# Black-Phoenix/CUDA-SfM

Hardware: AMD Instinct MI355X
Metric: RANSAC E-matrix hypotheses/sec (8-point, fused scoring), inlier-mask parity vs CPU oracle (higher is better)
Workload: dtype f32

## Files before the change

### cuda-sfm_amd/csrc/prefilter_lds.hpp

```cpp
#pragma once
#include "prefilter_record.hpp"

namespace sfm {

constexpr int kPfTileMax = 1024;
constexpr int kPfWaves = 16;
constexpr int kPfRing = 128;

constexpr int kPfERow = 10;
constexpr int kPfWaveBytes = 32 * kPfERow * 4 + 32 * 4;
template <int RULE> struct PfLds {
    static constexpr int kFragsPerBlock = RULE == kPfRuleG ? 3 : 2;
    static constexpr int kBlockBytes = kFragsPerBlock * 64 * 16;
    static constexpr int kFrag = 0;
    static constexpr int kTileMax = kPfTileMax;
    int staged, pts, ring, wave, next, lut, bytes;
    __host__ __device__ explicit PfLds(int tile, int ring_entries = kPfRing, int entry_bytes = 8)
    {
        staged = (tile + 63) & ~63;
        pts = kFrag + (staged / 32) * kBlockBytes;
        ring = pts + staged * 16;
        ring = (ring + ring_entries * entry_bytes - 1) & ~(ring_entries * entry_bytes - 1);
        wave = ring + kPfWaves * ring_entries * entry_bytes;
        next = wave + kPfWaves * kPfWaveBytes;
        lut = next + 16;
        bytes = lut + 32;
    }
};
static_assert(kPfRing * 8 == 1024, "ring slots are addressed with (offset & 1023) | base");

static inline int pf_tile_points(int ld, int tmax)
{
    const int ntiles = (ld + tmax - 1) / tmax;
    const int t = ((ld + ntiles - 1) / ntiles + 31) & ~31;
    return t < 32 ? 32 : t;
}

}
```

### cuda-sfm_amd/csrc/ransac_prefilter.hip

```cpp
#include "ransac_device.hpp"
#include "block_ops.hpp"
#include "prefilter_math.hpp"
#include "prefilter_record.hpp"
#include "prefilter_lds.hpp"

namespace sfm {

typedef float f16v __attribute__((ext_vector_type(16)));


__device__ constexpr int kPfESlot[9] = { 2, 6, 1, 3, 5, 7, 0, 4, 8 };
__device__ __forceinline__ uint32_t shift_in_reject(uint32_t rejected, float nt, float G)
{
    return __builtin_amdgcn_alignbit(rejected, __float_as_uint(fmaf(-nt, nt, G)), 31);
}

__device__ __forceinline__ uint32_t scan16(const f16v &nt, const f16v &G)
{
    uint32_t rejected = 0u;
#pragma unroll
    for (int r = 0; r < 16; ++r) rejected = shift_in_reject(rejected, nt[r], G[r]);
    return rejected;
}

__device__ __forceinline__ uint32_t scan16_band(const f16v &nt)
{
    uint32_t w = 0u;
#pragma unroll
    for (int r = 0; r < 16; ++r) w = __builtin_amdgcn_alignbit(w, __float_as_uint(nt[r]), 30);
    return w;
}

typedef uint32_t u6v __attribute__((ext_vector_type(6)));
constexpr uint32_t kPackM0 = 0x10410410u, kPackM1 = 0x04104104u;

__device__ __forceinline__ uint32_t pf_bfi(uint32_t m, uint32_t a, uint32_t b) { return __builtin_amdgcn_bitop3_b32(m, a, b, 0xCA); }

__device__ __forceinline__ uint32_t pack_reject_bits(const u6v &d)
{
    const uint32_t wa = pf_bfi(kPackM0 | kPackM1, pf_bfi(kPackM0, d[0], d[1]), d[2]);
    const uint32_t wb = pf_bfi(kPackM0 | kPackM1, pf_bfi(kPackM0, d[3], d[4]), d[5]);
    return pf_bfi(0x55555555u, wa, wb << 1);
}

typedef uint32_t u2v __attribute__((ext_vector_type(2)));
typedef float f4v __attribute__((ext_vector_type(4)));
typedef __attribute__((address_space(3))) u2v lds_u2;
typedef uint32_t u4v __attribute__((ext_vector_type(4)));
typedef __attribute__((address_space(3))) u4v lds_u4;
typedef __attribute__((address_space(3))) const f4v lds_cf4;
typedef __attribute__((address_space(3))) const float lds_cf;
typedef __attribute__((address_space(3))) int lds_i;
typedef __attribute__((address_space(3))) const h8 lds_ch8;
typedef __attribute__((address_space(3))) const v2f lds_cv2;
typedef __attribute__((address_space(3))) const unsigned char lds_cu8;

struct PfFrags { h8 n0, n1, t; };

__device__ __forceinline__ bool pf_exact_inlier(v2f p0, v2f p1, v2f p2, v2f p3, float e8, v2f xu, v2f yv, const ThrBand &band)
{
    const v2f e00 = { p3.x, p3.x }, e44 = { p3.y, p3.y }, e31 = { p1.y, p1.x };
    const v2f ab0 = __builtin_elementwise_fma(p1, yv, __builtin_elementwise_fma(e00, xu, p0));
    const v2f ab1 = __builtin_elementwise_fma(e44, yv, __builtin_elementwise_fma(e31, xu, p2));
    const float a2 = fmaf(p2.y, yv.x, fmaf(p0.y, xu.x, e8));
    const float nn = fmaf(yv.y, ab1.x, fmaf(xu.y, ab0.x, a2));
    const float n2 = nn * nn;
    const v2f dd = __builtin_elementwise_fma(ab1, ab1, ab0 * ab0);
    const float da = dd.x, db = dd.y;
    const float m = n2 * (da + db);
    const float tp = (da * db) * band.thr;
    const uint32_t mb = __float_as_uint(m), tb = __float_as_uint(tp);
    const uint32_t gap = __usad(mb, tb, 0u);
    const bool undecided = (gap < kBandUlps) || (tb < band.lo_bits) || (tb > band.hi_bits);
    bool in = m < tp;
    if (undecided) {
        const float t1 = (da == 0.0f) ? 0.0f : n2 / da;
        const float t2 = (db == 0.0f) ? 0.0f : n2 / db;
        in = (t1 + t2) < band.thr;
    }
    return in;
}

template <int RULE>
__device__ __forceinline__ PfFrags load_point_frags(lds_ch8 *frag_lane, int pb)
{
    lds_ch8 *p = frag_lane + pb * (PfLds<RULE>::kBlockBytes / 16);
    if (RULE != kPfRuleG) return PfFrags{ p[0], p[64], h8{} };
    return PfFrags{ p[0], p[64], p[128] };
}

template <int RULE>
__device__ __forceinline__ void mfma_step(const PfFrags &a, const PfFrags &b, f16v &G, f16v &nt)
{
    const f16v z = {};
    nt = __builtin_amdgcn_mfma_f32_32x32x16_f16(a.n0, b.n0, z, 0, 0, 0);
    if (RULE == kPfRuleG) G = __builtin_amdgcn_mfma_f32_32x32x16_f16(a.t, b.t, z, 0, 0, 0);
    nt = __builtin_amdgcn_mfma_f32_32x32x16_f16(a.n1, b.n1, nt, 0, 0, 0);
}

#define PF_SCHED_STEP()                                                 \
    do {                                                                \
        if (RULE != kPfRuleG) {                                         \
            __builtin_amdgcn_sched_group_barrier(0x008, 1, 0);          \
            __builtin_amdgcn_sched_group_barrier(0x002, 8, 0);          \
            __builtin_amdgcn_sched_group_barrier(0x008, 1, 0);          \
            __builtin_amdgcn_sched_group_barrier(0x002, 8, 0);          \
        } else {                                                        \
            __builtin_amdgcn_sched_group_barrier(0x008, 1, 0);          \
            __builtin_amdgcn_sched_group_barrier(0x002, 11, 0);         \
            __builtin_amdgcn_sched_group_barrier(0x008, 1, 0);          \
            __builtin_amdgcn_sched_group_barrier(0x002, 11, 0);         \
            __builtin_amdgcn_sched_group_barrier(0x008, 1, 0);          \
            __builtin_amdgcn_sched_group_barrier(0x002, 11, 0);         \
        }                                                               \
    } while (0)

constexpr int kPfVarTickets = 1;

constexpr int pf_score_waves_per_simd(int var, int rule, int fl2, int pipe, int wide, int prio)
{
    return (var == 0 && (rule == kPfRuleBandTile || rule == kPfRuleBandPack) && !fl2 && !pipe && !wide && !prio) ? 5 : 4;
}

template <int W, int VAR = 0, int RULE = kPfRuleBandTile, int FL2 = 0, int PIPE = 0, int WIDE = 0, int PRIO = 0>
__global__ __launch_bounds__(W * 64, pf_score_waves_per_simd(VAR, RULE, FL2, PIPE, WIDE, PRIO))
void ransac_score_prefilter(const float *__restrict__ X0, const float *__restrict__ X1, int ld, int n,
                            const float *__restrict__ Ecand, const PfRecord *__restrict__ recs, uint32_t h0, uint32_t count, float thr,
                            int dynamic, int tile,
                            int *__restrict__ counts, uint32_t *__restrict__ tick,
                            unsigned long long *best_key, unsigned long long *best_key2, unsigned long long *__restrict__ clk,
                            const unsigned long long *__restrict__ bound_word, const uint32_t *__restrict__ tile_boxes)
{
    extern __shared__ __attribute__((aligned(16))) unsigned char smem[];
    const int lane = threadIdx.x & 63;
    const int wave = __builtin_amdgcn_readfirstlane(threadIdx.x >> 6);
    const bool probe = clk && blockIdx.x == 0 && blockIdx.y == 0 && threadIdx.x == 0;
    unsigned long long c0 = 0, w0 = 0;
    if (clk && blockIdx.x == 0 && blockIdx.y == 0 && wave == 0) { c0 = clock64(); w0 = wall_clock64(); }
#if SFM_AB
    const uint32_t trace_blk = blockIdx.y * gridDim.x + blockIdx.x;
    unsigned long long *trace = (clk && trace_blk < (uint32_t)kTraceBlocks) ? clk + 8 + (size_t)trace_blk * kTraceWords : nullptr;
    if (trace && threadIdx.x == 0) {
        trace[0] = wall_clock64();
        trace[2] = ((unsigned long long)__builtin_amdgcn_s_getreg((20 << 0) | (0 << 6) | (31 << 11)) << 32) |
                   (unsigned long long)__builtin_amdgcn_s_getreg((4 << 0) | (0 << 6) | (31 << 11));
        trace[3] = ((unsigned long long)blockIdx.y << 32) | blockIdx.x;
    }
#define PF_PHASE(k) do { if (probe1) clk[k] = wall_clock64() - w0; } while (0)
#else
#define PF_PHASE(k) do { } while (0)
#endif
    const int half = lane >> 5, row = lane & 31;
    const uint32_t npass = (count + (uint32_t)kPfGroup - 1u) / (uint32_t)kPfGroup;
    const uint32_t nstatic = gridDim.x * (uint32_t)W;
    using LT = PfLds<RULE>;
    constexpr bool kBand = RULE != kPfRuleG, kTile = RULE == kPfRuleBandTile, kPack = RULE == kPfRuleBandPack || kTile;
    static_assert(!(FL2 && kPack) && !(VAR && kPack), "the recorded variants were built on the v_alignbit scan");
    constexpr int kRing = FL2 ? 256 : kPfRing;
    constexpr int kEnt = WIDE ? 16 : 8;
    static_assert(!WIDE || (kPack && !PIPE && !FL2), "wide entries: the packed scan's plain loop only");
    const LT L(tile, kRing, kEnt);
    float *etab = reinterpret_cast<float *>(smem + L.wave + wave * kPfWaveBytes);
    int *cnt = reinterpret_cast<int *>(etab + 32 * kPfERow);

    PfFrags afrag = {};
    uint32_t key0 = 0u;
    float rec_dn = 0.0f, rec_lin = 0.0f;
    float e_row[9] = {};
    auto fetch_pass = [&](uint32_t pass, PfFrags &af, uint32_t &k0, float (&e)[9], float &dn, float &lin) {
        const uint32_t hf = pass * (uint32_t)kPfGroup;
        const uint32_t h = hf + (uint32_t)min(row, (int)min((uint32_t)kPfGroup, count - hf) - 1);
        if (kTile) {
            const float *src = Ecand + 9 * (size_t)h;
#pragma unroll
            for (int k = 0; k < 9; ++k) e[k] = src[k];
            const uint4 rec = reinterpret_cast<const uint4 *>(recs)[h];
            k0 = rec.x; dn = __uint_as_float(rec.y); lin = __uint_as_float(rec.z);
            return;
        }
        const uint4 *r = reinterpret_cast<const uint4 *>(recs + h) + 2 * half;
        const uint4 r0 = r[0], r1 = r[1];
        if (kBand) pf_band_record_expand(r0, r1, half, af.n0, af.n1, k0);
        else pf_record_expand(r0, r1, half, af.n0, af.n1, af.t, k0);
        if (half == 0) {
            const float *src = Ecand + 9 * (size_t)h;
#pragma unroll
            for (int k = 0; k < 9; ++k) e[k] = src[k];
        }
    };
    auto install_rows = [&](const float (&e)[9]) {
        if (half == 0) {
#pragma unroll
            for (int k = 0; k < 9; ++k) etab[32 * k + row] = e[kPfESlot[k]];
            cnt[row] = 0;
        }
    };
    uint32_t ps = blockIdx.x * (uint32_t)W + (uint32_t)wave;
    bool have = ps < npass;
    if (have) { fetch_pass(ps, afrag, key0, e_row, rec_dn, rec_lin); install_rows(e_row); }

    SFM_PHASE("stage_tile");
    uint32_t *next_idx = reinterpret_cast<uint32_t *>(smem + L.next);
    if (threadIdx.x == 0) *next_idx = (uint32_t)W;
    if (kPack && threadIdx.x < 32) smem[L.lut + threadIdx.x] = (unsigned char)pf_pack_code((int)threadIdx.x);
    float pf_B = 0.0f;
    uint32_t bw[8] = {};
    uint32_t bw_lane = 0u;
    if (kTile) {
        pf_B = __uint_as_float((uint32_t)(__hip_atomic_load(reinterpret_cast<const uint32_t *>(bound_word), __ATOMIC_RELAXED, __HIP_MEMORY_SCOPE_AGENT)));
        bw_lane = __hip_atomic_load(tile_boxes + 8 * blockIdx.y + (lane & 7), __ATOMIC_RELAXED, __HIP_MEMORY_SCOPE_AGENT);
    }
    __syncthreads();
    const int tile_first = blockIdx.y * tile;
    for (int t = threadIdx.x; t < L.staged; t += W * 64) {
        const int p = tile_first + t;
        float u = 0.f, v = 0.f, x = 0.f, y = 0.f;
        const bool real = p < n && t < tile;
        if (kTile) {
            if (real) {
                const float4 q4 = reinterpret_cast<const float4 *>(X0)[p];
                u = q4.x; v = q4.y; x = q4.z; y = q4.w;
            }
        } else
        if (real) { u = X0[p]; v = X0[(size_t)ld + p]; x = X1[p]; y = X1[(size_t)ld + p]; }
        _Float16 bn[kPfSlots], bt[kPfSlotsT];
        prefilter_point_slots(u, v, x, y, real, bn, bt);
        reinterpret_cast<float4 *>(smem + L.pts)[t] = real ? make_float4(x, u, y, v) : make_float4(NAN, NAN, NAN, NAN);
        const int pb = t >> 5, col = t & 31;
        unsigned char *blk = smem + LT::kFrag + pb * LT::kBlockBytes;
#pragma unroll
        for (int ks = 0; ks < 2; ++ks)
#pragma unroll
            for (int hh = 0; hh < 2; ++hh) {
                h8 c;
#pragma unroll
                for (int j = 0; j < 8; ++j) c[j] = bn[ks * 16 + hh * 8 + j];
                *reinterpret_cast<h8 *>(blk + ks * 1024 + (hh * 32 + col) * 16) = c;
            }
        if (RULE == kPfRuleG) {
#pragma unroll
            for (int hh = 0; hh < 2; ++hh) {
                h8 c;
#pragma unroll
                for (int j = 0; j < 8; ++j) c[j] = bt[hh * 8 + j];
                *reinterpret_cast<h8 *>(blk + 2048 + (hh * 32 + col) * 16) = c;
            }
        }
    }
    __syncthreads();
    PfBox tbox = {};
    auto build_operands = [&](const float (&e)[9], uint32_t fl, float dn, float lin) {
        int half_l = half;
        float thr_l = thr, B_l = pf_B;
        asm volatile("" : "+v"(half_l), "+s"(thr_l), "+s"(B_l));
        pf_tile_operands(e, fl, dn, lin, thr_l, B_l, tbox, half_l, afrag.n0, afrag.n1);
        key0 = fl & kPfTileFlagScan;
    };
    if (kTile) {
#pragma unroll
        for (int k = 0; k < 8; ++k) bw[k] = (uint32_t)__builtin_amdgcn_readlane((int)bw_lane, k);
        pf_B = uniform(pf_B);
        tbox = pf_box_from_bits(bw, pf_B);
        tbox = PfBox{ uniform(tbox.xlo), uniform(tbox.xhi), uniform(tbox.ylo), uniform(tbox.yhi), uniform(tbox.ulo), uniform(tbox.uhi), uniform(tbox.vlo), uniform(tbox.vhi) };
        if (have) build_operands(e_row, key0, rec_dn, rec_lin);
    }
#if SFM_AB
    if (probe) clk[2] = wall_clock64() - w0;
#endif
    const int npb = (min(tile, ld - tile_first) + 31) >> 5;
    const int npp = (npb + 1) >> 1;
    const float4 *pts = reinterpret_cast<const float4 *>(smem + L.pts);
    lds_cf *etab_l = (lds_cf *)etab;
    lds_i *cnt_l = (lds_i *)cnt;
    lds_cu8 *lut_l = (lds_cu8 *)(smem + L.lut);
    const uint32_t ring_base = (uint32_t)(size_t)(__attribute__((address_space(3))) unsigned char *)(smem + L.ring) + (uint32_t)wave * (uint32_t)(kRing * kEnt);
    uint32_t ring_mask = (uint32_t)(kRing * kEnt - 1);
    asm("" : "+v"(ring_mask));
    auto ring_at = [&](uint32_t index8) {
        return (lds_u2 *)((__attribute__((address_space(3))) unsigned char *)0 + ((index8 & ring_mask) | ring_base));
    };
    auto ring_at16 = [&](uint32_t index16) {
        return (lds_u4 *)((__attribute__((address_space(3))) unsigned char *)0 + ((index16 & ring_mask) | ring_base));
    };
    lds_ch8 *frag_lane = (lds_ch8 *)(smem + LT::kFrag) + lane;
    const ThrBand band = make_band(thr);
    uint32_t passes_done = 0;

    while (have) {
        SFM_PHASE("pass_begin");
        const uint32_t h_first = ps * (uint32_t)kPfGroup;
        const int nvalid = (int)min((uint32_t)kPfGroup, count - h_first);
#if SFM_AB
        const bool probe1 = probe && passes_done == 0u;
#endif
        uint32_t ps_next = ps + nstatic;
        if (dynamic) {
            uint32_t got = 0u;
            if (lane == 0) got = atomicAdd(next_idx, 1u);
            got = (uint32_t)__builtin_amdgcn_readfirstlane((int)got);
            ps_next = (got / (uint32_t)W) * nstatic + blockIdx.x * (uint32_t)W + (got % (uint32_t)W);
        }
        {
            const bool scan = key0 != 0u;
            const unsigned long long sm = __ballot(scan);
            uint32_t todo = (uint32_t)sm | (uint32_t)(sm >> 32);
            uint32_t survive = 0u;
            while (todo) {
                const int r = __builtin_ctz(todo);
                todo &= todo - 1u;
                const float se[6] = { etab[6 * 32 + r], etab[2 * 32 + r], etab[r], etab[3 * 32 + r], etab[7 * 32 + r], etab[4 * 32 + r] };
                bool z = false;
                for (int j = 0; j < L.staged / 64; ++j) {
                    const float4 q = pts[j * 64 + lane];
                    z = z || prefilter_zero_divisor(se, q.x, q.z);
                }
                if (__ballot(z) != 0ull) survive |= 1u << r;
            }
            if (survive != 0u && ((survive >> row) & 1u)) {
                const h8 zero = {};
                afrag.n0 = zero; afrag.n1 = zero; afrag.t = zero;
                if (half) { afrag.n1[3] = (_Float16)1.0f; afrag.t[7] = (_Float16)0.0009765625f; }
            }
        }
        PF_PHASE(3);

        int head = 0, nq = 0;
        const uint32_t lane_tag = (uint32_t)(size_t)(lds_cf4 *)pts + (uint32_t)(row * 16) + (uint32_t)(half * 4);
        auto flush = [&](int m) {
            uint32_t rest = 0, tag = 0;
            if (PRIO == 2) __builtin_amdgcn_s_setprio(2);
            if (lane < m) {
                const u2v ent = *ring_at(((uint32_t)head + (uint32_t)lane) * 8u);
                tag = ent.y;
                const uint32_t surv = ent.x;
                const int b = __builtin_clz(surv);
                rest = surv & ~(0x80000000u >> b);
                int hl, sub;
                if (kPack) {
                    const uint32_t code = lut_l[b];
                    hl = (int)(code & 31u) + (int)(tag & 4u); sub = (int)(code >> 5);
                } else {
                    const int r = kBand ? b >> 1 : b & 15;
                    sub = kBand ? b & 1 : b >> 4;
                    hl = r + (r & 12) + (int)(tag & 4u);
                }
                if (hl < nvalid) {
                    const f4v q = *(lds_cf4 *)((__attribute__((address_space(3))) const unsigned char *)0 + ((tag & ~15u) + ((uint32_t)sub << 9)));
                    lds_cf *e = etab_l + hl;
                    const v2f p0 = { e[0], e[32] }, p1 = { e[64], e[96] }, p2 = { e[128], e[160] }, p3 = { e[192], e[224] };
                    const float e8 = e[256];
                    if (pf_exact_inlier(p0, p1, p2, p3, e8, v2f{ q.x, q.y }, v2f{ q.z, q.w }, band))
                        __hip_atomic_fetch_add(cnt_l + hl, 1, __ATOMIC_RELAXED, __HIP_MEMORY_SCOPE_WORKGROUP);
                }
            }
            const unsigned long long more = __ballot(rest != 0u);
            if (more) {
                const int slot = __builtin_amdgcn_mbcnt_hi((uint32_t)(more >> 32), __builtin_amdgcn_mbcnt_lo((uint32_t)more, 0u));
                if (rest) *ring_at(((uint32_t)(head + nq) + (uint32_t)slot) * 8u) = u2v{ rest, tag };
            }
            head = (head + m) & (kRing - 1);
            nq += __builtin_popcountll(more) - m;
            if (PRIO == 2) __builtin_amdgcn_s_setprio(0);
        };
        auto flush_w = [&](int m) {
            uint32_t ra = 0, rb = 0, tag = 0;
            if (lane < m) {
                const u4v ent = *ring_at16(((uint32_t)head + (uint32_t)lane) * 16u);
                tag = ent.z;
                const bool second = ent.x == 0u;
                const uint32_t surv = second ? ent.y : ent.x;
                const int b = __builtin_clz(surv);
                const uint32_t left = surv & ~(0x80000000u >> b);
                ra = second ? 0u : left; rb = second ? left : ent.y;
                const uint32_t code = lut_l[b];
                const int hl = (int)(code & 31u) + (int)(tag & 4u);
                if (hl < nvalid) {
                    const f4v q = *(lds_cf4 *)((__attribute__((address_space(3))) const unsigned char *)0 + ((tag & ~15u) + ((code >> 5) << 9) + (second ? 1024u : 0u)));
                    lds_cf *e = etab_l + hl;
                    const v2f p0 = { e[0], e[32] }, p1 = { e[64], e[96] }, p2 = { e[128], e[160] }, p3 = { e[192], e[224] };
                    const float e8 = e[256];
                    if (pf_exact_inlier(p0, p1, p2, p3, e8, v2f{ q.x, q.y }, v2f{ q.z, q.w }, band))
                        __hip_atomic_fetch_add(cnt_l + hl, 1, __ATOMIC_RELAXED, __HIP_MEMORY_SCOPE_WORKGROUP);
                }
            }
            const unsigned long long more = __ballot((ra | rb) != 0u);
            if (more) {
                const int slot = __builtin_amdgcn_mbcnt_hi((uint32_t)(more >> 32), __builtin_amdgcn_mbcnt_lo((uint32_t)more, 0u));
                if ((ra | rb) != 0u) *ring_at16(((uint32_t)(head + nq) + (uint32_t)slot) * 16u) = u4v{ ra, rb, tag, 0u };
            }
            head = (head + m) & (kRing - 1);
            nq += __builtin_popcountll(more) - m;
        };
        auto flush2 = [&]() {
            const u2v entA = *ring_at(((uint32_t)head + (uint32_t)lane) * 8u), entB = *ring_at(((uint32_t)head + 64u + (uint32_t)lane) * 8u);
            const int bA = __builtin_clz(entA.x), bB = __builtin_clz(entB.x);
            const uint32_t restA = entA.x & ~(0x80000000u >> bA), restB = entB.x & ~(0x80000000u >> bB);
            const int rA = bA >> 1, rB = bB >> 1;
            const int hlA = rA + (rA & 12) + (int)(entA.y & 4u), hlB = rB + (rB & 12) + (int)(entB.y & 4u);
            const int hcA = min(hlA, nvalid - 1), hcB = min(hlB, nvalid - 1);
            const f4v qA = *(lds_cf4 *)((__attribute__((address_space(3))) const unsigned char *)0 + ((entA.y & ~15u) + ((uint32_t)(bA & 1) << 9)));
            const f4v qB = *(lds_cf4 *)((__attribute__((address_space(3))) const unsigned char *)0 + ((entB.y & ~15u) + ((uint32_t)(bB & 1) << 9)));
            lds_cf *eA = etab_l + hcA, *eB = etab_l + hcB;
            const v2f a0 = { eA[0], eA[32] }, a1 = { eA[64], eA[96] }, a2 = { eA[128], eA[160] }, a3 = { eA[192], eA[224] };
            const float a8 = eA[256];
            const v2f b0 = { eB[0], eB[32] }, b1 = { eB[64], eB[96] }, b2 = { eB[128], eB[160] }, b3 = { eB[192], eB[224] };
            const float b8 = eB[256];
            const bool inA = pf_exact_inlier(a0, a1, a2, a3, a8, v2f{ qA.x, qA.y }, v2f{ qA.z, qA.w }, band);
            const bool inB = pf_exact_inlier(b0, b1, b2, b3, b8, v2f{ qB.x, qB.y }, v2f{ qB.z, qB.w }, band);
            if (inA && hlA < nvalid) __hip_atomic_fetch_add(cnt_l + hlA, 1, __ATOMIC_RELAXED, __HIP_MEMORY_SCOPE_WORKGROUP);
            if (inB && hlB < nvalid) __hip_atomic_fetch_add(cnt_l + hlB, 1, __ATOMIC_RELAXED, __HIP_MEMORY_SCOPE_WORKGROUP);
            const unsigned long long moreA = __ballot(restA != 0u), moreB = __ballot(restB != 0u);
            if (moreA | moreB) {
                const int nA = __builtin_popcountll(moreA);
                const int slotA = __builtin_amdgcn_mbcnt_hi((uint32_t)(moreA >> 32), __builtin_amdgcn_mbcnt_lo((uint32_t)moreA, 0u));
                const int slotB = nA + __builtin_amdgcn_mbcnt_hi((uint32_t)(moreB >> 32), __builtin_amdgcn_mbcnt_lo((uint32_t)moreB, 0u));
                if (restA) *ring_at(((uint32_t)(head + nq) + (uint32_t)slotA) * 8u) = u2v{ restA, entA.y };
                if (restB) *ring_at(((uint32_t)(head + nq) + (uint32_t)slotB) * 8u) = u2v{ restB, entB.y };
            }
            head = (head + 128) & (kRing - 1);
            nq += __builtin_popcountll(moreA) + __builtin_popcountll(moreB) - 128;
        };

        if constexpr (kPack && PIPE) {
        PfFrags fa = load_point_frags<RULE>(frag_lane, 0), fb = load_point_frags<RULE>(frag_lane, 1);
        lds_ch8 *fp = frag_lane + 2 * (LT::kBlockBytes / 16);
        const f16v zero16 = {};
        f16v a0, a1, b0, b1;
        a0 = __builtin_amdgcn_mfma_f32_32x32x16_f16(afrag.n0, fa.n0, zero16, 0, 0, 0);
        a1 = __builtin_amdgcn_mfma_f32_32x32x16_f16(afrag.n0, fb.n0, zero16, 0, 0, 0);
        a0 = __builtin_amdgcn_mfma_f32_32x32x16_f16(afrag.n1, fa.n1, a0, 0, 0, 0);
        a1 = __builtin_amdgcn_mfma_f32_32x32x16_f16(afrag.n1, fb.n1, a1, 0, 0, 0);
        fa = load_point_frags<RULE>(fp, 0);
        fb = load_point_frags<RULE>(fp, 1);
        fp += 2 * (LT::kBlockBytes / 16);
        auto phase = [&](const f16v &c0, const f16v &c1, f16v &m0, f16v &m1, int pp) {
            SFM_PHASE("scan_two_steps");
            __builtin_amdgcn_sched_barrier(0);
            m0 = __builtin_amdgcn_mfma_f32_32x32x16_f16(afrag.n0, fa.n0, zero16, 0, 0, 0);
            __builtin_amdgcn_sched_barrier(0);
            const u6v d = __builtin_amdgcn_cvt_scalef32_2xpk16_bf6_f32(c0, c1, 1.0f);
            __builtin_amdgcn_sched_barrier(0);
            m1 = __builtin_amdgcn_mfma_f32_32x32x16_f16(afrag.n0, fb.n0, zero16, 0, 0, 0);
            __builtin_amdgcn_sched_barrier(0);
            const uint32_t rej32 = pack_reject_bits(d);
            __builtin_amdgcn_sched_barrier(0);
            m0 = __builtin_amdgcn_mfma_f32_32x32x16_f16(afrag.n1, fa.n1, m0, 0, 0, 0);
            __builtin_amdgcn_sched_barrier(0);
            const bool mine = rej32 != 0xFFFFFFFFu;
            const unsigned long long any = __ballot(mine);
            __builtin_amdgcn_sched_barrier(0);
            m1 = __builtin_amdgcn_mfma_f32_32x32x16_f16(afrag.n1, fb.n1, m1, 0, 0, 0);
            __builtin_amdgcn_sched_barrier(0);
            fa = load_point_frags<RULE>(fp, 0);
            fb = load_point_frags<RULE>(fp, 1);
            fp += 2 * (LT::kBlockBytes / 16);
            __builtin_amdgcn_sched_barrier(0);
            SFM_PHASE("append_and_inloop_flush");
            if (any) {
                while (nq >= 64) flush(64);
                const int slot = __builtin_amdgcn_mbcnt_hi((uint32_t)(any >> 32), __builtin_amdgcn_mbcnt_lo((uint32_t)any, 0u));
                if (mine) *ring_at(((uint32_t)(head + nq) + (uint32_t)slot) * 8u) = u2v{ ~rej32, lane_tag + ((uint32_t)pp << 10) };
                nq += __builtin_popcountll(any);
            }
        };
        for (int pp = 0; pp < npp; pp += 2) {
            phase(a0, a1, b0, b1, pp);
            if (pp + 1 < npp) phase(b0, b1, a0, a1, pp + 1);
        }
        } else if constexpr (kPack) {
        PfFrags fa = load_point_frags<RULE>(frag_lane, 0), fb = load_point_frags<RULE>(frag_lane, 1);
        lds_ch8 *fp = frag_lane + 2 * (LT::kBlockBytes / 16);
        f16v g0, n0, n1;
        u6v dpk = {};
        auto append = [&](const u6v &d, int pp) {
            const uint32_t rej32 = pack_reject_bits(d);
            const bool mine = rej32 != 0xFFFFFFFFu;
            const unsigned long long any = __ballot(mine);
            SFM_PHASE("append_and_inloop_flush");
            if (any) {
                while (nq >= 64) flush(64);
                const int slot = __builtin_amdgcn_mbcnt_hi((uint32_t)(any >> 32), __builtin_amdgcn_mbcnt_lo((uint32_t)any, 0u));
                if (mine) *ring_at(((uint32_t)(head + nq) + (uint32_t)slot) * 8u) = u2v{ ~rej32, lane_tag + ((uint32_t)pp << 10) };
                nq += __builtin_popcountll(any);
            }
        };
        uint32_t rej_even = 0xFFFFFFFFu;
        auto append_w = [&](uint32_t ra, uint32_t rb, int pp_even) {
            const bool mine = (ra & rb) != 0xFFFFFFFFu;
            const unsigned long long any = __ballot(mine);
            if (any) {
                while (nq >= 64) flush_w(64);
                const int slot = __builtin_amdgcn_mbcnt_hi((uint32_t)(any >> 32), __builtin_amdgcn_mbcnt_lo((uint32_t)any, 0u));
                if (mine) *ring_at16(((uint32_t)(head + nq) + (uint32_t)slot) * 16u) = u4v{ ~ra, ~rb, lane_tag + ((uint32_t)pp_even << 10), 0u };
                nq += __builtin_popcountll(any);
            }
        };
        auto after_phase = [&](const u6v &d, int pp) {
            if (!WIDE) { append(d, pp); return; }
            const uint32_t rej32 = pack_reject_bits(d);
            if ((pp & 1) == 0) rej_even = rej32;
            else append_w(rej_even, rej32, pp - 1);
        };
        for (int pp = 0; pp < npp; ++pp) {
            SFM_PHASE("scan_two_steps");
            if (PRIO == 1) __builtin_amdgcn_s_setprio(2);
            mfma_step<RULE>(afrag, fa, g0, n0);
            mfma_step<RULE>(afrag, fb, g0, n1);
            fa = load_point_frags<RULE>(fp, 0);
            fb = load_point_frags<RULE>(fp, 1);
            fp += 2 * (LT::kBlockBytes / 16);
            if (PRIO == 1) __builtin_amdgcn_s_setprio(0);
            __builtin_amdgcn_sched_barrier(0);
            if (pp > 0) after_phase(dpk, pp - 1);
            __builtin_amdgcn_sched_barrier(0);
            dpk = __builtin_amdgcn_cvt_scalef32_2xpk16_bf6_f32(n0, n1, 1.0f);
            __builtin_amdgcn_sched_barrier(0);
        }
        after_phase(dpk, npp - 1);
        if (WIDE && (npp & 1)) append_w(rej_even, 0xFFFFFFFFu, npp - 1);
        } else {
        PfFrags fa = load_point_frags<RULE>(frag_lane, 0), fb = load_point_frags<RULE>(frag_lane, 1);
        f16v g0, n0, g1, n1;
        mfma_step<RULE>(afrag, fa, g0, n0);
        lds_ch8 *fp = frag_lane + 2 * (LT::kBlockBytes / 16);
        for (int pp = 0; pp < npp; ++pp) {
            SFM_PHASE("scan_two_steps");
            fa = load_point_frags<RULE>(fp, 0);
            __builtin_amdgcn_sched_barrier(0);
            mfma_step<RULE>(afrag, fb, g1, n1);
            const uint32_t rej_first = kBand ? scan16_band(n0) : scan16(n0, g0);
            PF_SCHED_STEP();
            __builtin_amdgcn_sched_barrier(0);
            fb = load_point_frags<RULE>(fp, 1);
            fp += 2 * (LT::kBlockBytes / 16);
            __builtin_amdgcn_sched_barrier(0);
            mfma_step<RULE>(afrag, fa, g0, n0);
            const uint32_t rej_second = kBand ? scan16_band(n1) : scan16(n1, g1);
            PF_SCHED_STEP();
            __builtin_amdgcn_sched_barrier(0);
            const uint32_t rej32 = kBand ? (((rej_first << 1) & 0xAAAAAAAAu) | (rej_second & 0x55555555u))
                                                       : ((rej_first << 16) | rej_second);
            const bool mine = rej32 != 0xFFFFFFFFu;
            const unsigned long long any = __ballot(mine);
            SFM_PHASE("append_and_inloop_flush");
            if (any) {
                if (FL2) { while (nq >= 128) flush2(); }
                else
                while (nq >= 64) flush(64);
                const int slot = __builtin_amdgcn_mbcnt_hi((uint32_t)(any >> 32), __builtin_amdgcn_mbcnt_lo((uint32_t)any, 0u));
                if (mine) *ring_at(((uint32_t)(head + nq) + (uint32_t)slot) * 8u) = u2v{ ~rej32, lane_tag + ((uint32_t)pp << 10) };
                nq += __builtin_popcountll(any);
            }
        }
        }
        PF_PHASE(4);
        SFM_PHASE("pass_end_fetch_next");
        const bool have_next = ps_next < npass;
        PfFrags afrag_next = afrag;
        uint32_t key0n = 0u;
        float e_next[9] = {}, dn_next = 0.0f, lin_next = 0.0f;
        if (have_next) fetch_pass(ps_next, afrag_next, key0n, e_next, dn_next, lin_next);
        SFM_PHASE("drain_flush");
        if (FL2) { while (nq >= 128) flush2(); }
        if (WIDE) { while (nq > 0) flush_w(min(nq, 64)); }
        while (nq > 0) flush(min(nq, 64));
        SFM_PHASE("epilogue");
        PF_PHASE(7);
        if (VAR & kPfVarTickets) {
        if (lane < nvalid) {
            const int c = cnt[lane];
            if (c) atomicAdd(&counts[h_first + lane], c);
        }
        asm volatile("s_waitcnt vmcnt(0)" ::: "memory");
        uint32_t t = 0;
        if (lane == 0) t = atomicAdd(&tick[ps], 1u);
        t = __builtin_amdgcn_readfirstlane(t);
        if (t == gridDim.y - 1) {
            unsigned long long k = 0;
            if (lane < nvalid) {
                const int c = __hip_atomic_load(&counts[h_first + lane], __ATOMIC_RELAXED, __HIP_MEMORY_SCOPE_AGENT);
                k = pack_key((uint32_t)c, h0 + h_first + (uint32_t)lane);
            }
            k = wave_max(k);
            if (lane == 0 && k) {
                atomicMax(best_key, k);
                if (best_key2) atomicMax(best_key2, k);
            }
        }
        } else {
        uint32_t c_mine = 0u;
        unsigned long long old = 0ull;
        if (lane < nvalid) {
            c_mine = (uint32_t)cnt[lane];
            unsigned long long *acc = reinterpret_cast<unsigned long long *>(tick) + (h_first + (uint32_t)lane);
            old = atomicAdd(acc, (1ull << 32) | (unsigned long long)c_mine);
        }
        const int nvalid_done = nvalid;
        const uint32_t h_done = h_first;
        if (have_next) {
            if (kTile) build_operands(e_next, key0n, dn_next, lin_next);
            else { afrag = afrag_next; key0 = key0n; }
            install_rows(e_next);
        }
        unsigned long long k = 0;
        if (lane < nvalid_done && (uint32_t)(old >> 32) == gridDim.y - 1u) {
            const uint32_t total = (uint32_t)old + c_mine;
            counts[h_done + lane] = (int)total;
            k = pack_key(total, h0 + h_done + (uint32_t)lane);
        }
        if (__ballot(k != 0ull) != 0ull) {
            k = wave_max(k);
            if (lane == 0 && k > __hip_atomic_load(best_key, __ATOMIC_RELAXED, __HIP_MEMORY_SCOPE_AGENT)) {
                atomicMax(best_key, k);
                if (best_key2) atomicMax(best_key2, k);
            }
        }
        }
        PF_PHASE(5);
        ++passes_done;
        have = have_next;
        if (have_next) {
            ps = ps_next;
            if (VAR & kPfVarTickets) { afrag = afrag_next; key0 = key0n; install_rows(e_next); }
        }
    }
    SFM_PHASE("kernel_end");
    if (probe) { clk[6] = passes_done; clk[0] = clock64() - c0; clk[1] = wall_clock64() - w0; }
#if SFM_AB
    if (trace && lane == 0) {
        const unsigned long long tend = wall_clock64();
        trace[4 + wave] = tend;
        if (wave == 0) trace[1] = tend;
    }
#endif
}

constexpr int kPfBuckets = 1024 + 2;
constexpr int kPfBucketBlock = 256;

__device__ __forceinline__ int pf_bucket_of(const float4 q, float B)
{
    const float big = fmaxf(fmaxf(fabsf(q.x), fabsf(q.y)), fmaxf(fabsf(q.z), fabsf(q.w)));
    if (!(big <= 48.0f) || q.x != q.x || q.y != q.y || q.z != q.z || q.w != q.w) return kPfBuckets - 2;
    return (int)(pf_morton_key(q.x, q.y, -B, B, -B, B) >> 20);
}

__global__ __launch_bounds__(1024)
void pf_bucket_scan_kernel(uint32_t *__restrict__ hist, int nblocks, uint32_t *__restrict__ base, uint32_t *__restrict__ boxes, int nbox_words)
{
    for (int k = threadIdx.x; k < nbox_words; k += blockDim.x) boxes[k] = pf_order_bits(-INFINITY);
    __shared__ uint32_t total[kPfBuckets + 1024];
    for (int b = threadIdx.x; b < kPfBuckets; b += blockDim.x) {
        uint32_t run = 0u;
        for (int k = 0; k < nblocks; ++k) {
            const uint32_t c = hist[(size_t)k * kPfBuckets + b];
            hist[(size_t)k * kPfBuckets + b] = run;
            run += c;
        }
        total[b] = run;
    }
    __syncthreads();
    __shared__ uint32_t wsum[17];
    base[threadIdx.x] = block_scan<16>(total[threadIdx.x], wsum);
    if (threadIdx.x == 0) { base[1024] = wsum[16]; base[1025] = wsum[16] + total[1024]; }
}
static_assert(kPfBuckets == 1026, "pf_bucket_scan_kernel: 1024 Morton buckets scanned by 1024 threads + two special ones");

constexpr int kPfBoxTilesLds = 512;
__global__ __launch_bounds__(kPfBucketBlock)
void pf_bucket_scatter_kernel(const float4 *__restrict__ pts4, int n, int ld, const unsigned long long *__restrict__ bound_word,
                              const uint32_t *__restrict__ hist, const uint32_t *__restrict__ base, float4 *__restrict__ out,
                              int tile, int ntiles, uint32_t *__restrict__ boxes)
{
    constexpr int kWaves = kPfBucketBlock / 64;
    __shared__ unsigned short hw[kWaves][kPfBuckets];
    extern __shared__ uint32_t bx[];
    const int nlds = min(ntiles, kPfBoxTilesLds);
    for (int k = threadIdx.x; k < kWaves * kPfBuckets; k += blockDim.x) (&hw[0][0])[k] = 0;
    for (int k = threadIdx.x; k < nlds * 8; k += blockDim.x) bx[k] = pf_order_bits(-INFINITY);
    __syncthreads();
    const float B = __uint_as_float((uint32_t)(*bound_word & 0xFFFFFFFFull));
    const int i = blockIdx.x * kPfBucketBlock + threadIdx.x, lane = threadIdx.x & 63, wave = threadIdx.x >> 6;
    float4 q = make_float4(0.f, 0.f, 0.f, 0.f);
    int bucket = -1;
    if (i < n) { q = pts4[i]; bucket = pf_bucket_of(q, B); }
    int below = 0, same = 0;
    for (int j = 0; j < 64; ++j) {
        const int bj = __builtin_amdgcn_readlane(bucket, j);
        below += (bj == bucket && j < lane) ? 1 : 0;
        same += (bj == bucket) ? 1 : 0;
    }
    if (bucket >= 0 && below == same - 1) hw[wave][bucket] = (unsigned short)same;
    __syncthreads();
    if (i >= n) {
        if (i < ld) out[i] = pts4[i];
    } else {
        uint32_t earlier = 0u;
        for (int w = 0; w < wave; ++w) earlier += hw[w][bucket];
        const uint32_t dest = base[bucket] + hist[(size_t)blockIdx.x * kPfBuckets + bucket] + earlier + (uint32_t)below;
        out[dest] = q;
        if (bucket != kPfBuckets - 2) {
            const int t = (int)dest / tile;
            const float ext[8] = { q.z, -q.z, q.w, -q.w, q.x, -q.x, q.y, -q.y };
            uint32_t *w = t < nlds ? bx + 8 * t : boxes + 8 * (size_t)t;
#pragma unroll
            for (int k = 0; k < 8; ++k) atomicMax(w + k, pf_order_bits(ext[k]));
        }
    }
    __syncthreads();
    for (int k = threadIdx.x; k < nlds * 8; k += blockDim.x) {
        const uint32_t v = bx[k];
        if (v != pf_order_bits(-INFINITY)) atomicMax(boxes + k, v);
    }
}

__global__ __launch_bounds__(256)
void pf_cells_build_kernel(const float4 *__restrict__ pts4, int n, unsigned long long *__restrict__ bound_word,
                           uint32_t *__restrict__ cells, uint32_t mask, uint32_t epoch, uint32_t *__restrict__ hist)
{
    static_assert(kPfBucketBlock == 256, "one histogram per block of this kernel");
    __shared__ uint32_t bh[kPfBuckets];
    if (hist) {
        for (int b = threadIdx.x; b < kPfBuckets; b += blockDim.x) bh[b] = 0u;
        __syncthreads();
    }
    const int j = blockIdx.x * blockDim.x + threadIdx.x;
    float4 q = make_float4(0.f, 0.f, 0.f, 0.f);
    bool feat = false;
    if (j < n) {
        q = pts4[j];
        const float big = fmaxf(fmaxf(fabsf(q.x), fabsf(q.y)), fmaxf(fabsf(q.z), fabsf(q.w)));
        feat = big <= 48.0f && q.x == q.x && q.y == q.y && q.z == q.z && q.w == q.w;
    }
    float ext[8] = { q.z, -q.z, q.w, -q.w, q.x, -q.x, q.y, -q.y };
#pragma unroll
    for (int k = 0; k < 8; ++k) {
        if (!feat) ext[k] = -INFINITY;
#pragma unroll
        for (int off = 32; off > 0; off >>= 1) ext[k] = fmaxf(ext[k], __shfl_xor(ext[k], off));
    }
    if (cells && (threadIdx.x & 63) == 0) {
#pragma unroll
        for (int k = 0; k < 8; ++k) atomicMax(bound_word + 2 + k, ((unsigned long long)epoch << 32) | pf_order_bits(ext[k]));
    }
    const float Bq = __uint_as_float((uint32_t)(*bound_word & 0xFFFFFFFFull));
    if (hist) {
        if (j < n) atomicAdd(&bh[pf_bucket_of(q, Bq)], 1u);
        __syncthreads();
        for (int b = threadIdx.x; b < kPfBuckets; b += blockDim.x) hist[(size_t)blockIdx.x * kPfBuckets + b] = bh[b];
    }
    if (!feat || !cells) return;
    const PfGrid grid = prefilter_grid(Bq);
#pragma unroll
    for (int side = 0; side < 2; ++side) {
        const uint32_t key = side ? pf_cell_key_side(pf_cell(q.x, grid), pf_cell(q.y, grid), 1) : pf_cell_key(pf_cell(q.z, grid), pf_cell(q.w, grid));
        uint32_t sl = pf_cells_slot(key, mask);
        for (;;) {
            const uint32_t old = atomicCAS(&cells[sl], 0u, key);
            if (old == 0u || old == key) break;
            sl = (sl + 1) & mask;
        }
    }
}

int launch_pf_cells(sfm_pair *pair, bool want_sorted, int tile)
{
    hipStream_t st = pair->ctx->stream;
    const bool cells_ok = pair->cells_epoch == pair->bound_epoch && pair->d_cells;
    const bool order_ok = !want_sorted || (pair->sorted_epoch == pair->bound_epoch && pair->boxes_tile == tile && pair->d_pts4s);
    if (cells_ok && st != pair->cells_stream) SFM_HIP_TRY(hipStreamWaitEvent(st, pair->cells_ev, 0));
    if (cells_ok && order_ok) return SFM_OK;
    if (!cells_ok) {
        uint32_t slots = 4096;
        while (slots < 8u * (uint32_t)pair->n) slots <<= 1;
        const int rcg = grow(&pair->d_cells, &pair->cells_cap, slots, st);
        if (rcg != SFM_OK) return rcg;
        pair->cells_mask = slots - 1u;
        SFM_HIP_TRY(hipMemsetAsync(pair->d_cells, 0, (size_t)slots * sizeof(uint32_t), st));
    }
    const int nblk = (pair->n + kPfBucketBlock - 1) / kPfBucketBlock;
// ... 117 lines not shown
        for (int k = 0; k < 16; ++k) { out[32 + k] = (float)ts[k]; out[80 + k] = (float)bt[k]; }
        out[96] = accn[0]; out[97] = accg[0];
        out[98] = (float)(shift_in_reject(0u, accn[0], accg[0]) & 1u);
        int cx0, cx1, cy0, cy1;
        out[99] = (float)prefilter_zero_divisor_cells(e, B, prefilter_grid(B), cx0, cx1, cy0, cy1);
    }
}

__global__ __launch_bounds__(64)
void pf_band_probe_kernel(const float *__restrict__ E, float thr, float B, PfBox box, int b_safe, float u, float v, float x, float y, int survive_all,
                          PfRecord *rec, float *__restrict__ out)
{
    const int lane = threadIdx.x;
    const int half = lane >> 5;
    float e[9];
#pragma unroll
    for (int k = 0; k < 9; ++k) e[k] = E[k];
    const bool pack = (b_safe & 2) != 0;
    const float sigma = survive_all ? 0.0f : prefilter_band_sigma(e, thr, B, box, (b_safe & 1) != 0, pack ? kPfBandTopPack : kPfBandTop);
    if (lane == 0) pf_band_store(e, sigma, false, rec);
    __threadfence();
    __syncthreads();
    _Float16 ns[kPfSlots], bn[kPfSlots], bt[kPfSlotsT];
    {
        const volatile uint4 *vr = reinterpret_cast<const volatile uint4 *>(rec);
        uint4 w[4];
#pragma unroll
        for (int q = 0; q < 4; ++q) { w[q].x = vr[q].x; w[q].y = vr[q].y; w[q].z = vr[q].z; w[q].w = vr[q].w; }
#pragma unroll
        for (int hh = 0; hh < 2; ++hh) {
            h8 f0, f1; uint32_t fl;
            pf_band_record_expand(w[2 * hh], w[2 * hh + 1], hh, f0, f1, fl);
#pragma unroll
            for (int j = 0; j < 8; ++j) { ns[hh * 8 + j] = f0[j]; ns[16 + hh * 8 + j] = f1[j]; }
        }
    }
    prefilter_point_slots(u, v, x, y, true, bn, bt);
    h8 an0, an1, b0, b1;
#pragma unroll
    for (int j = 0; j < 8; ++j) {
        an0[j] = half ? ns[8 + j] : ns[j];   an1[j] = half ? ns[24 + j] : ns[16 + j];
        b0[j] = half ? bn[8 + j] : bn[j];    b1[j] = half ? bn[24 + j] : bn[16 + j];
    }
    f16v accn = {};
    accn = __builtin_amdgcn_mfma_f32_32x32x16_f16(an0, b0, accn, 0, 0, 0);
    accn = __builtin_amdgcn_mfma_f32_32x32x16_f16(an1, b1, accn, 0, 0, 0);
    if (lane == 0) {
        for (int k = 0; k < 32; ++k) { out[k] = (float)ns[k]; out[48 + k] = (float)bn[k]; }
        out[96] = accn[0]; out[97] = sigma;
        f16v one = {}; one[0] = accn[0];
        out[98] = (float)((scan16_band(one) >> 30) & 1u);
        if (pack) {
            f16v far = {};
#pragma unroll
            for (int k = 0; k < 16; ++k) far[k] = 256.0f;
            f16v s0 = far; s0[0] = accn[0];
            const uint32_t rej = pack_reject_bits(__builtin_amdgcn_cvt_scalef32_2xpk16_bf6_f32(s0, far, 1.0f));
            out[98] = (float)((~rej) == 0u);
        }
        int cx0, cx1, cy0, cy1;
        out[99] = (float)prefilter_zero_divisor_cells(e, B, prefilter_grid(B), cx0, cx1, cy0, cy1);
        float et[9];
        prefilter_transposed(e, et);
        out[100] = (float)prefilter_zero_divisor_cells(et, B, prefilter_grid(B), cx0, cx1, cy0, cy1);
    }
    {
        const int j = (lane & 31) >> 1, st = lane & 1;
        f16v s0, s1;
#pragma unroll
        for (int k = 0; k < 16; ++k) { s0[k] = (k == j && st == 0) ? u : 256.0f; s1[k] = (k == j && st == 1) ? u : 256.0f; }
        const uint32_t surv = ~pack_reject_bits(__builtin_amdgcn_cvt_scalef32_2xpk16_bf6_f32(s0, s1, 1.0f));
        bool ok;
        if (prefilter_band_pack_reject(u)) ok = surv == 0u;
        else {
            const int b = __builtin_clz(surv | 1u);
            ok = surv != 0u && (surv & (surv - 1u)) == 0u && pf_pack_code(b) == ((uint32_t)((j & 3) + 8 * (j >> 2)) | ((uint32_t)st << 5));
        }
        const unsigned long long okm = __ballot(ok && lane < 32);
        if (lane == 0) { out[101] = (float)__builtin_popcountll(okm); out[102] = (float)(surv == 0u); }
    }
}

int launch_prefilter_band_probe(sfm_ctx *ctx, const float *d_E, float thr, float B, const float box[8], int b_safe, const float pt[4], int survive_all, float *d_out)
{
    const PfBox bx = { box[0], box[1], box[2], box[3], box[4], box[5], box[6], box[7] };
    hipLaunchKernelGGL(pf_band_probe_kernel, dim3(1), dim3(64), 0, ctx->stream, d_E, thr, B, bx, b_safe, pt[0], pt[1], pt[2], pt[3], survive_all,
                       reinterpret_cast<PfRecord *>(d_out + 128), d_out);
    SFM_HIP_TRY(hipGetLastError());
    return SFM_OK;
}

int launch_prefilter_probe(sfm_ctx *ctx, const float *d_E, float thr, float B, const float pt[4], int survive_all, float *d_out)
{
    PfScales sc;
    if (!prefilter_scales(thr, sc)) { set_error("threshold %g outside the pre-filter's range", (double)thr); return SFM_E_INVALID; }
    hipLaunchKernelGGL(pf_probe_kernel, dim3(1), dim3(64), 0, ctx->stream, d_E, thr, B, sc, pt[0], pt[1], pt[2], pt[3], survive_all,
                       reinterpret_cast<PfRecord *>(d_out + 128), d_out);
    SFM_HIP_TRY(hipGetLastError());
    return SFM_OK;
}
#endif

static int pf_rule_switch(const sfm_ransac_params &p)
{
    if (SFM_SW(p, 3) == 4 || SFM_SW(p, 3) >= 16) return kPfRuleG;
    if (SFM_SW(p, 3) == 5 || SFM_SW(p, 1) == 5 || SFM_SW(p, 1) == 7 || SFM_SW(p, 1) == 9) return kPfRuleBand;
    if (SFM_SW(p, 3) == 6 || SFM_SW(p, 1) == 11 || SFM_SW(p, 1) == 12) return kPfRuleBandPack;
    if (SFM_SW(p, 3) == 7 || SFM_SW(p, 1) == 13 || SFM_SW(p, 1) == 14 || SFM_SW(p, 1) == 15) return kPfRuleBandTile;
    return -1;
}

constexpr uint64_t kPfOrderFirstCallPairs = 1ull << 33;
int prefilter_pick_rule(sfm_pair *pair, const sfm_ransac_params &p, uint32_t count)
{
    int rule = pf_rule_switch(p);
    if (rule < 0) {
        const bool ordered = pair->sorted_epoch == pair->bound_epoch && pair->d_pts4s != nullptr;
        const bool first = pair->pf_seen_epoch != pair->bound_epoch;
        rule = (!ordered && first && (uint64_t)count * (uint64_t)pair->ld < kPfOrderFirstCallPairs) ? kPfRuleBandPack : kPfRuleBandTile;
    }
    pair->pf_seen_epoch = pair->bound_epoch;
    pair->pf_rule = rule;
    return rule;
}

bool prefilter_usable(const sfm_pair *pair, const sfm_ransac_params &p, uint32_t count)
{
    PfScales sc;
    return pair->state.unit_z && pair->state.have_bound && count >= 16384u && (uint64_t)count * (uint64_t)pair->ld >= (1ull << 27) && prefilter_scales(p.threshold, sc);
}

static int pf_tile_of(const sfm_pair *pair, const sfm_ransac_params &p)
{
    if (SFM_SW(p, 1) == 7 && pair->pf_rule == kPfRuleBand) return pf_tile_points(pair->ld, 1536);
    return pf_tile_points(pair->ld, kPfTileMax);
}

int prefilter_tile_points(const sfm_pair *pair, const sfm_ransac_params &p) { return pf_tile_of(pair, p); }

int launch_score_prefilter(sfm_pair *pair, const sfm_ransac_params &p, uint32_t h0, uint32_t count, unsigned long long *key2)
{
    sfm_ctx *ctx = pair->ctx;
    PfScales sc;
    if (!prefilter_scales(p.threshold, sc)) { set_error("threshold %g outside the pre-filter's range", (double)p.threshold); return SFM_E_INVALID; }
    const int waves = (SFM_SW(p, 1) == 5 || SFM_SW(p, 1) == 12) ? 12 : kPfWaves;
    const int tile = pf_tile_of(pair, p);
    const int ntiles = (pair->ld + tile - 1) / tile;
    const uint32_t npass = (count + (uint32_t)kPfGroup - 1u) / (uint32_t)kPfGroup;
    const uint32_t iters = (npass + (uint32_t)waves - 1) / (uint32_t)waves;
    uint32_t cols = (uint32_t)ctx->num_cus / (uint32_t)ntiles;
    if (SFM_SW(p, 2) > 0) cols = (uint32_t)SFM_SW(p, 2);
    if (cols > iters) cols = iters;
    if (cols < 1) cols = 1;
    const int dynamic = SFM_SW(p, 1) == 2 ? 0 : 1;
    const int var = SFM_SW(p, 3) >= 16 ? SFM_SW(p, 3) - 16 : 0;
    const int rule = pair->pf_rule;
    const bool fl2 = rule == kPfRuleBand && waves == kPfWaves && SFM_SW(p, 1) == 9;
    const bool wide = rule == kPfRuleBandTile && SFM_SW(p, 1) == 13;
    const int lds_bytes = wide ? PfLds<kPfRuleBand>(tile, kPfRing, 16).bytes : fl2 ? PfLds<kPfRuleBand>(tile, 256).bytes : rule != kPfRuleG ? PfLds<kPfRuleBand>(tile).bytes : PfLds<kPfRuleG>(tile).bytes;
    if (lds_bytes > 160 * 1024) { set_error("pre-filter tile of %d points needs %d bytes of LDS", tile, lds_bytes); return SFM_E_INVALID; }
    auto launch = [&](auto kernel) -> int {
        const int rc_lds = allow_big_lds(ctx, reinterpret_cast<const void *>(kernel));
        if (rc_lds != SFM_OK) return rc_lds;
        const float *x0 = rule == kPfRuleBandTile ? reinterpret_cast<const float *>(pair->d_pts4s) : pair->d_X[0];
        hipLaunchKernelGGL(kernel, dim3(cols, ntiles), dim3(waves * 64), lds_bytes, ctx->stream,
                           x0, pair->d_X[1], pair->ld, pair->n, pair->d_Ecand, reinterpret_cast<const PfRecord *>(pair->d_pf), h0, count, p.threshold,
                           dynamic, tile, pair->d_counts, pair->d_tick, pair->d_key, key2, pair->d_clk, pair->d_bound, pair->d_tile_boxes);
        return SFM_OK;
    };
    int rcl;
#if SFM_AB
    if (rule == kPfRuleG && waves == 12) rcl = launch(&ransac_score_prefilter<12, 0, kPfRuleG>);
    else if (rule == kPfRuleG && var == 1) rcl = launch(&ransac_score_prefilter<16, 1, kPfRuleG>);
    else if (rule == kPfRuleG) rcl = launch(&ransac_score_prefilter<16, 0, kPfRuleG>);
    else if (waves == 12) rcl = launch(&ransac_score_prefilter<12, 0, kPfRuleBand>);
    else if (fl2) rcl = launch(&ransac_score_prefilter<16, 0, kPfRuleBand, 1>);
    else if (rule == kPfRuleBand) rcl = launch(&ransac_score_prefilter<16, 0, kPfRuleBand>);
    else if (SFM_SW(p, 1) == 11) rcl = launch(&ransac_score_prefilter<16, 0, kPfRuleBandPack, 0, 1>);
    else if (SFM_SW(p, 1) == 12) rcl = launch(&ransac_score_prefilter<12, 0, kPfRuleBandPack, 0, 1>);
    else if (wide) rcl = launch(&ransac_score_prefilter<16, 0, kPfRuleBandTile, 0, 0, 1>);
    else if (rule == kPfRuleBandTile && SFM_SW(p, 1) == 14) rcl = launch(&ransac_score_prefilter<16, 0, kPfRuleBandTile, 0, 0, 0, 1>);
    else if (rule == kPfRuleBandTile && SFM_SW(p, 1) == 15) rcl = launch(&ransac_score_prefilter<16, 0, kPfRuleBandTile, 0, 0, 0, 2>);
    else
#endif
    if (rule == kPfRuleBandPack) rcl = launch(&ransac_score_prefilter<16, 0, kPfRuleBandPack>);
    else rcl = launch(&ransac_score_prefilter<16, 0, kPfRuleBandTile>);
    (void)var; (void)fl2; (void)wide;
    if (rcl != SFM_OK) return rcl;
    SFM_HIP_TRY(hipGetLastError());
    pair->last_grid = (int)cols * ntiles; pair->last_block = waves * 64; pair->last_lds = lds_bytes;
    return SFM_OK;
}

}
```

### profiles/phase_probe.py

```python
import json
import os
import sys

sys.path.insert(0, os.path.dirname(os.path.dirname(os.path.abspath(__file__))))
import numpy as np
import torch
import cuda_sfm_amd_ab as S
from cuda_sfm_amd_ab import synth

dev = torch.device("cuda", 0)
ctx = S.Context(0, torch.cuda.current_stream().cuda_stream)
n = 4096
scene = synth.two_view_scene(n)
d_sift = torch.from_numpy(scene["sift"].view(np.uint8).reshape(n, 576)).to(dev)
pair = S.ImagePair(ctx, scene["K"], scene["Kinv"], 2, n)
pair.fillXU(d_sift)
for H, cols in ((131072, 0), (131072, 64), (262144, 0), (1048576, 0), (1048576, 64)):
    p = S.default_params(n, num_hypotheses=H, seed=3, kernel=S.KERNEL_PREFILTER)
    p.reserved[2] = cols
    for _ in range(10):
        pair.estimateE(p)
    ctx.kernel_timing(True) if hasattr(ctx, "kernel_timing") else None
    pair.estimateE(p)
    t = pair.last_phases()
    us = lambda k: round(t[k] / 100.0, 2)
    print(json.dumps({"hypotheses": H, "grid": pair.last_launch()["grid"], "block0_lifetime_us": us(1), "tile_staged_us": us(2), "first_pass_prepared_us": us(3),
                      "first_block_scanned_us": us(4), "ring_drained_us": us(7), "first_pass_done_us": us(5), "passes_of_wave0": t[6],
                      "shader_mhz": round(100.0 * t[0] / max(t[1], 1))}), flush=True)
```

Measured before the change: 2.732 billion.

## Fan out ring tail drain across lanes and batch best-key updates per block

```diff
diff --git a/cuda-sfm_amd/csrc/prefilter_lds.hpp b/cuda-sfm_amd/csrc/prefilter_lds.hpp
--- a/cuda-sfm_amd/csrc/prefilter_lds.hpp
+++ b/cuda-sfm_amd/csrc/prefilter_lds.hpp
@@ -14,7 +14,7 @@
     static constexpr int kBlockBytes = kFragsPerBlock * 64 * 16;
     static constexpr int kFrag = 0;
     static constexpr int kTileMax = kPfTileMax;
-    int staged, pts, ring, wave, next, lut, bytes;
+    int staged, pts, ring, wave, next, lut, key, bytes;
     __host__ __device__ explicit PfLds(int tile, int ring_entries = kPfRing, int entry_bytes = 8)
     {
         staged = (tile + 63) & ~63;
@@ -24,7 +24,8 @@
         wave = ring + kPfWaves * ring_entries * entry_bytes;
         next = wave + kPfWaves * kPfWaveBytes;
         lut = next + 16;
-        bytes = lut + 32;
+        key = lut + 32;
+        bytes = key + 8;
     }
 };
 static_assert(kPfRing * 8 == 1024, "ring slots are addressed with (offset & 1023) | base");
diff --git a/cuda-sfm_amd/csrc/ransac_prefilter.hip b/cuda-sfm_amd/csrc/ransac_prefilter.hip
--- a/cuda-sfm_amd/csrc/ransac_prefilter.hip
+++ b/cuda-sfm_amd/csrc/ransac_prefilter.hip
@@ -54,6 +54,7 @@
 typedef __attribute__((address_space(3))) const h8 lds_ch8;
 typedef __attribute__((address_space(3))) const v2f lds_cv2;
 typedef __attribute__((address_space(3))) const unsigned char lds_cu8;
+typedef __attribute__((address_space(3))) unsigned long long lds_u64;
 
 struct PfFrags { h8 n0, n1, t; };
 
@@ -146,9 +147,15 @@
                    (unsigned long long)__builtin_amdgcn_s_getreg((4 << 0) | (0 << 6) | (31 << 11));
         trace[3] = ((unsigned long long)blockIdx.y << 32) | blockIdx.x;
     }
-#define PF_PHASE(k) do { if (probe1) clk[k] = wall_clock64() - w0; } while (0)
+    const int probe_sel = dynamic >> 8;
+    dynamic &= 0xFF;
+#define PF_PROBE_SEL probe_sel
+#define PF_PHASE(k) do { if (probe1 && ((k) != 3 || !probe_sel)) clk[k] = wall_clock64() - w0; } while (0)
+#define PF_TAIL(k) do { if (probe1 && probe_sel) clk[k] = wall_clock64() - w0; } while (0)
 #else
+#define PF_PROBE_SEL 0
 #define PF_PHASE(k) do { } while (0)
+#define PF_TAIL(k) do { } while (0)
 #endif
     const int half = lane >> 5, row = lane & 31;
     const uint32_t npass = (count + (uint32_t)kPfGroup - 1u) / (uint32_t)kPfGroup;
@@ -159,6 +166,7 @@
     constexpr int kRing = FL2 ? 256 : kPfRing;
     constexpr int kEnt = WIDE ? 16 : 8;
     static_assert(!WIDE || (kPack && !PIPE && !FL2), "wide entries: the packed scan's plain loop only");
+    constexpr bool kTail = VAR == 0 && kPack && !FL2 && !PIPE && !WIDE && !PRIO;
     const LT L(tile, kRing, kEnt);
     float *etab = reinterpret_cast<float *>(smem + L.wave + wave * kPfWaveBytes);
     int *cnt = reinterpret_cast<int *>(etab + 32 * kPfERow);
@@ -201,7 +209,8 @@
 
     SFM_PHASE("stage_tile");
     uint32_t *next_idx = reinterpret_cast<uint32_t *>(smem + L.next);
-    if (threadIdx.x == 0) *next_idx = (uint32_t)W;
+    lds_u64 *blk_key = (lds_u64 *)(smem + L.key);
+    if (threadIdx.x == 0) { *next_idx = (uint32_t)W; *blk_key = 0ull; }
     if (kPack && threadIdx.x < 32) smem[L.lut + threadIdx.x] = (unsigned char)pf_pack_code((int)threadIdx.x);
     float pf_B = 0.0f;
     uint32_t bw[8] = {};
@@ -291,8 +300,9 @@
         const uint32_t h_first = ps * (uint32_t)kPfGroup;
         const int nvalid = (int)min((uint32_t)kPfGroup, count - h_first);
 #if SFM_AB
-        const bool probe1 = probe && passes_done == 0u;
+        const bool probe1 = probe && passes_done == (uint32_t)(probe_sel ? probe_sel - 1 : 0);
 #endif
+        PF_TAIL(2);
         uint32_t ps_next = ps + nstatic;
         if (dynamic) {
             uint32_t got = 0u;
@@ -362,6 +372,42 @@
             nq += __builtin_popcountll(more) - m;
             if (PRIO == 2) __builtin_amdgcn_s_setprio(0);
         };
+        auto flush_fan = [&]() {
+            const int g = min(64 / nq, 8);
+            const int k = (int)(((float)lane + 0.5f) * __builtin_amdgcn_rcpf((float)nq));
+            const int ei = lane - k * nq;
+            uint32_t left = 0, tag = 0;
+            if (k < g) {
+                const u2v ent = *ring_at(((uint32_t)head + (uint32_t)ei) * 8u);
+                tag = ent.y;
+                uint32_t r = __builtin_bitreverse32(ent.x), mine = 0u;
+                for (int j = 0; j < g; ++j) {
+                    if (j == k) mine = r;
+                    r &= r - 1u;
+                }
+                if (k == 0) left = r;
+                if (mine != 0u) {
+                    const int b = __builtin_ctz(mine);
+                    const uint32_t code = lut_l[b];
+                    const int hl = (int)(code & 31u) + (int)(tag & 4u), sub = (int)(code >> 5);
+                    if (hl < nvalid) {
+                        const f4v q = *(lds_cf4 *)((__attribute__((address_space(3))) const unsigned char *)0 + ((tag & ~15u) + ((uint32_t)sub << 9)));
+                        lds_cf *e = etab_l + hl;
+                        const v2f p0 = { e[0], e[32] }, p1 = { e[64], e[96] }, p2 = { e[128], e[160] }, p3 = { e[192], e[224] };
+                        const float e8 = e[256];
+                        if (pf_exact_inlier(p0, p1, p2, p3, e8, v2f{ q.x, q.y }, v2f{ q.z, q.w }, band))
+                            __hip_atomic_fetch_add(cnt_l + hl, 1, __ATOMIC_RELAXED, __HIP_MEMORY_SCOPE_WORKGROUP);
+                    }
+                }
+            }
+            const unsigned long long more = __ballot(left != 0u);
+            if (more) {
+                const int slot = __builtin_amdgcn_mbcnt_hi((uint32_t)(more >> 32), __builtin_amdgcn_mbcnt_lo((uint32_t)more, 0u));
+                if (left) *ring_at(((uint32_t)(head + nq) + (uint32_t)slot) * 8u) = u2v{ __builtin_bitreverse32(left), tag };
+            }
+            head = (head + nq) & (kRing - 1);
+            nq = __builtin_popcountll(more);
+        };
         auto flush_w = [&](int m) {
             uint32_t ra = 0, rb = 0, tag = 0;
             if (lane < m) {
@@ -563,6 +609,10 @@
         SFM_PHASE("drain_flush");
         if (FL2) { while (nq >= 128) flush2(); }
         if (WIDE) { while (nq > 0) flush_w(min(nq, 64)); }
+        if (kTail) {
+            while (nq > 64) flush(64);
+            while (nq > 0) flush_fan();
+        } else
         while (nq > 0) flush(min(nq, 64));
         SFM_PHASE("epilogue");
         PF_PHASE(7);
@@ -602,13 +652,16 @@
             else { afrag = afrag_next; key0 = key0n; }
             install_rows(e_next);
         }
+        PF_TAIL(3);
         unsigned long long k = 0;
         if (lane < nvalid_done && (uint32_t)(old >> 32) == gridDim.y - 1u) {
             const uint32_t total = (uint32_t)old + c_mine;
             counts[h_done + lane] = (int)total;
             k = pack_key(total, h0 + h_done + (uint32_t)lane);
-        }
-        if (__ballot(k != 0ull) != 0ull) {
+            if (kTail) __hip_atomic_fetch_max(blk_key, k, __ATOMIC_RELAXED, __HIP_MEMORY_SCOPE_WORKGROUP);
+        }
+        PF_TAIL(6);
+        if (!kTail && __ballot(k != 0ull) != 0ull) {
             k = wave_max(k);
             if (lane == 0 && k > __hip_atomic_load(best_key, __ATOMIC_RELAXED, __HIP_MEMORY_SCOPE_AGENT)) {
                 atomicMax(best_key, k);
@@ -625,7 +678,17 @@
         }
     }
     SFM_PHASE("kernel_end");
-    if (probe) { clk[6] = passes_done; clk[0] = clock64() - c0; clk[1] = wall_clock64() - w0; }
+    if (kTail) {
+        __syncthreads();
+        if (threadIdx.x == 0) {
+            const unsigned long long k = *blk_key;
+            if (k != 0ull && k > __hip_atomic_load(best_key, __ATOMIC_RELAXED, __HIP_MEMORY_SCOPE_AGENT)) {
+                atomicMax(best_key, k);
+                if (best_key2) atomicMax(best_key2, k);
+            }
+        }
+    }
+    if (probe) { if (!PF_PROBE_SEL) clk[6] = passes_done; clk[0] = clock64() - c0; clk[1] = wall_clock64() - w0; }
 #if SFM_AB
     if (trace && lane == 0) {
         const unsigned long long tend = wall_clock64();
@@ -1049,7 +1112,8 @@
     if (SFM_SW(p, 2) > 0) cols = (uint32_t)SFM_SW(p, 2);
     if (cols > iters) cols = iters;
     if (cols < 1) cols = 1;
-    const int dynamic = SFM_SW(p, 1) == 2 ? 0 : 1;
+    int dynamic = SFM_SW(p, 1) == 2 ? 0 : 1;
+    if (SFM_SW(p, 0) >= 256) dynamic |= (SFM_SW(p, 0) - 255) << 8;
     const int var = SFM_SW(p, 3) >= 16 ? SFM_SW(p, 3) - 16 : 0;
     const int rule = pair->pf_rule;
     const bool fl2 = rule == kPfRuleBand && waves == kPfWaves && SFM_SW(p, 1) == 9;
diff --git a/profiles/phase_probe.py b/profiles/phase_probe.py
--- a/profiles/phase_probe.py
+++ b/profiles/phase_probe.py
@@ -27,3 +27,22 @@
     print(json.dumps({"hypotheses": H, "grid": pair.last_launch()["grid"], "block0_lifetime_us": us(1), "tile_staged_us": us(2), "first_pass_prepared_us": us(3),
                       "first_block_scanned_us": us(4), "ring_drained_us": us(7), "first_pass_done_us": us(5), "passes_of_wave0": t[6],
                       "shader_mhz": round(100.0 * t[0] / max(t[1], 1))}), flush=True)
+
+for H in (1048576, 131072):
+    p = S.default_params(n, num_hypotheses=H, seed=3, kernel=S.KERNEL_PREFILTER)
+    for _ in range(10):
+        pair.estimateE(p)
+    passes = pair.last_phases()[6]
+    for third in (1, 3, 5):
+        k = max(1, passes * third // 6)
+        p.reserved[0] = 256 + k
+        rows = []
+        for _ in range(5):
+            pair.estimateE(p)
+            t = pair.last_phases()
+            rows.append([(t[j] - t[2]) / 100.0 for j in (4, 7, 3, 6, 5)] + [100.0 * t[0] / max(t[1], 1)])
+        rows.sort(key=lambda r: r[4])
+        r = rows[len(rows) // 2]
+        print(json.dumps({"hypotheses": H, "passes_of_wave0": passes, "pass": k, "scanned_us": round(r[0], 2), "ring_drained_us": round(r[1], 2),
+                          "next_installed_us": round(r[2], 2), "answer_used_us": round(r[3], 2), "key_handled_us": round(r[4], 2),
+                          "shader_mhz": round(r[5])}), flush=True)
```

Result: slower. 2.569 billion (-5.9%).
